# zetanumbers/myraytracer

Measured on AMD Instinct MI355X. Metric: Msamples/s (pixels x spp / s), random-spheres, higher is better.
Workload: dtype f32

## Files before the change

include/myraytracer_amd_debug.h:

```cpp
#ifndef MYRAYTRACER_AMD_DEBUG_H
#define MYRAYTRACER_AMD_DEBUG_H

#include "myraytracer_amd.h"

#ifdef __cplusplus
extern "C" {
#endif

int mrt_debug_srgb8_thresholds(float out[256]);
int mrt_debug_present_encode(mrt_ctx* ctx, const float* rgba, uint32_t width, uint32_t rows, int format, uint32_t flags,
                             uint8_t* out);
int mrt_debug_set_present_copy(mrt_ctx* ctx, int mode);
int mrt_debug_noise_reduce(mrt_ctx* ctx, const float* S, const float* rgba, uint32_t width, uint32_t rows, double K,
                           float threshold, float floor, mrt_noise_report* out, float* tiles_out);
int mrt_debug_denoise(mrt_ctx* ctx, const float* rgba, const float* S, double K, const float* guides, uint32_t width, uint32_t rows,
                      const mrt_denoise_params* params, float* out);
int mrt_debug_denoise_variance(mrt_ctx* ctx, const float* rgba, const float* S, double K, const float* guides, uint32_t width,
                               uint32_t rows, const mrt_denoise_params* params, uint32_t variance, float* out);
int mrt_debug_denoise_mix(mrt_ctx* ctx, const float* rgba, const float* S, double K, const float* guides, uint32_t width,
                          uint32_t rows, const mrt_denoise_params* params, uint32_t variance, const mrt_denoise_mix* mix, float* out);
int mrt_debug_read_guides(mrt_ctx* ctx, float* rays, int32_t* index, float* t, float* normal, float* albedo, size_t cap_pixels);
int mrt_debug_read_gathered_guides(mrt_ctx* root_ctx, float* rays, int32_t* index, float* t, float* normal, float* albedo, size_t cap_pixels);

int mrt_debug_set_gather_per_band(mrt_ctx* root_ctx, int enabled);
// ... 10 lines not shown
                          size_t boxes_cap, uint32_t info[8]);
int mrt_debug_build_boxes_top_down(const mrt_sphere* spheres, size_t n, uint32_t max_levels, uint32_t top_target, int open,
                                   float* boxes_out, size_t boxes_cap, uint32_t info[5]);
int mrt_debug_mfma_scale(double reach, float scale_out[4], uint32_t* neg_k2_bf16_pair_out);
int mrt_debug_build_sweep(const mrt_sphere* spheres, size_t n, const float* force_axis, float axis_out[3], float* records_out,
                          size_t records_cap, uint16_t* mfma_out, size_t mfma_cap, float origin_out[3], double* reach_out);
int mrt_debug_set_sweep_axes(mrt_ctx* ctx, const float* axis);
int mrt_debug_sweep_axes(mrt_ctx* ctx, float axis_out[3]);
int mrt_debug_world_hit(mrt_ctx* ctx, const float* rays, size_t n, int32_t* hit_out, uint32_t* candidates_out,
                        size_t cand_words_per_ray);
int mrt_debug_world_hit_stats(mrt_ctx* ctx, uint64_t out[2]);
int mrt_debug_arith(mrt_ctx* ctx, int mode, const uint32_t bits_range[4], uint64_t count, uint64_t seed, uint64_t out[3]);
int mrt_debug_arith_pairs(mrt_ctx* ctx, const float* x, const float* y, size_t n, uint32_t* out);
int mrt_debug_last_launch(mrt_ctx* ctx, uint32_t out[2]);
int mrt_debug_set_boxes(mrt_ctx* ctx, int mode);
int mrt_debug_sweep_variant(mrt_ctx* ctx);
int mrt_debug_set_frame_batching(mrt_ctx* ctx, int enabled);
int mrt_debug_set_tile_sort(mrt_ctx* ctx, int enabled);
int mrt_debug_sort_tiles(mrt_ctx* ctx, const uint32_t* cost, size_t n_cost, const uint32_t* list, size_t n, uint32_t* order_out);
#define MRT_TILE_ORDER_NONE 0u
#define MRT_TILE_ORDER_INDEX 1u
#define MRT_TILE_ORDER_SORTED 2u
#define MRT_TILE_ORDER_SORTED_LIST 3u
#define MRT_TILE_ORDER_LIST 4u
int mrt_debug_read_tile_schedule(mrt_ctx* ctx, uint32_t* cost_out, uint32_t* order_out, size_t cap, uint32_t* n_out,
                                 uint32_t info_out[4]);
int mrt_debug_set_schedule(mrt_ctx* ctx, uint32_t pilot_spp, int waves_per_cu);
int mrt_debug_lds_layout(uint32_t n_members, uint32_t n_nodes, uint32_t levels, uint32_t n_top_padded, uint32_t out[3]);
int mrt_debug_set_frames_in_flight(mrt_ctx* ctx, int slots);
int mrt_debug_width_policy(int op, const uint32_t workload[6], uint32_t state[7], double util, double rate);
// ... 36 lines not shown
```

myraytracer_amd/_lib.py:

```python
import ctypes as C
import importlib.util
import os
import sys

os.environ.setdefault("GPU_MAX_HW_QUEUES", "20")

_HERE = os.path.dirname(os.path.abspath(__file__))
LIB_PATH = os.environ.get("MRT_LIB_OVERRIDE") or os.path.join(_HERE, "lib", "libmyraytracer_amd.so")

EXPORTS = [
    "mrt_args_default", "mrt_args_resolve_size", "mrt_create", "mrt_destroy", "mrt_set_shard",
    "mrt_set_stream", "mrt_set_world_raw", "mrt_set_world", "mrt_update_spheres", "mrt_pack_world", "mrt_set_camera",
    "mrt_camera_derive", "mrt_set_seeds", "mrt_read_seeds", "mrt_redraw", "mrt_render", "mrt_sync",
    "mrt_reset", "mrt_get_locals", "mrt_set_rng_shuffle", "mrt_set_samples_per_frame", "mrt_set_rng_mode",
    "mrt_frames_done", "mrt_frame_weight", "mrt_frame_shuffle", "mrt_pixel_seed", "mrt_shard_info",
    "mrt_framebuffer_device_ptr", "mrt_read_framebuffer", "mrt_read_counters", "mrt_last_kernel_ms",
    "mrt_kernel_ms_history", "mrt_debug_read_counters", "mrt_debug_wave_log", "mrt_debug_set_tile_sort", "mrt_debug_set_cluster_factor", "mrt_debug_set_hierarchy", "mrt_debug_set_sweep", "mrt_debug_sweep_variant", "mrt_debug_build_hierarchy", "mrt_debug_read_pixel_costs", "mrt_debug_set_schedule", "mrt_debug_mfma_scale", "mrt_debug_build_sweep", "mrt_debug_set_sweep_axes", "mrt_debug_sweep_axes",
    "mrt_last_error", "mrt_status_string", "mrt_abi_version", "mrt_build_id", "mrt_scene_default", "mrt_scene_cover",
    "mrt_scene_stress", "mrt_scene_save", "mrt_scene_load", "mrt_write_pfm", "mrt_write_ppm",
    "mrt_srgb8", "mrt_write_png", "mrt_gather", "mrt_gather_rccl", "mrt_gathered_device_ptr", "mrt_read_gathered",
    "mrt_shard_global_row", "mrt_shard_local_rows", "mrt_unshard_rows", "mrt_debug_last_set_world_ms", "mrt_debug_world_hit", "mrt_debug_world_hit_stats", "mrt_debug_set_frame_batching", "mrt_debug_set_gather_per_band", "mrt_debug_arith", "mrt_debug_arith_pairs", "mrt_debug_set_boxes", "mrt_debug_build_boxes", "mrt_set_draw_counting", "mrt_debug_last_launch", "mrt_debug_set_frames_in_flight", "mrt_debug_lds_layout", "mrt_debug_build_boxes_top_down",
    "mrt_set_wait_timeout", "mrt_get_schedule", "mrt_set_schedule_hint", "mrt_debug_width_policy", "mrt_debug_stream_concurrency", "mrt_debug_wave_log_frame",
    "mrt_present", "mrt_present_acquire", "mrt_present_release", "mrt_set_present_ring", "mrt_debug_srgb8_thresholds",
    "mrt_debug_present_encode", "mrt_debug_set_present_copy",
# ... 5 lines not shown
    "mrt_debug_check_context", "mrt_debug_sort_tiles", "mrt_debug_read_tile_schedule", "mrt_debug_read_hierarchy",
    "mrt_regroup_spheres", "mrt_debug_regroup_info", "mrt_debug_set_regroup_block", "mrt_debug_pool_clusters",
    "mrt_debug_set_camera_masks", "mrt_debug_read_camera_masks", "mrt_debug_read_camera_lists",
    "mrt_temporal_params_default", "mrt_set_temporal", "mrt_get_temporal", "mrt_temporal_step", "mrt_temporal_reset",
    "mrt_read_temporal", "mrt_debug_read_temporal", "mrt_debug_load_temporal",
    "mrt_temporal_response_default", "mrt_set_temporal_response", "mrt_get_temporal_response",
    "mrt_debug_read_temporal_fast", "mrt_debug_load_temporal_fast",
    "mrt_set_gather_noise", "mrt_read_gathered_noise", "mrt_read_gathered_denoised", "mrt_debug_read_gathered_guides",
    "mrt_set_denoise_adaptive", "mrt_get_denoise_adaptive", "mrt_debug_load_accumulation",
    "mrt_auto_regroup_default", "mrt_set_auto_regroup", "mrt_get_auto_regroup", "mrt_read_regroup_stats",
    "mrt_denoise_mix_default", "mrt_set_denoise_mix", "mrt_get_denoise_mix", "mrt_debug_denoise_mix",
    "mrt_update_materials", "mrt_debug_material_shade",
    "mrt_debug_hold", "mrt_debug_hold_stamps",
    "mrt_noise_query_map", "mrt_budget_allocate", "mrt_render_budget",
    "mrt_noise_query_budget", "mrt_read_budget_plan", "mrt_render_planned", "mrt_debug_budget_plan",
]

PRESENT_RGBA8_SRGB, PRESENT_BGRA8_SRGB = 1, 2
PRESENT_FLIP_Y, PRESENT_GATHERED, PRESENT_DENOISED, PRESENT_TEMPORAL, PRESENT_GATHERED_DENOISED = 1, 2, 8, 16, 32
ACQUIRE_NEWEST, ACQUIRE_OLDEST = 0, 1
TILE_ORDER_KINDS = ("none", "index", "sorted", "sorted-list", "list")
DENOISE_VAR_ACCUMULATED, DENOISE_VAR_PREFILTERED, DENOISE_VAR_SPATIAL_EARLY = 0, 1, 2
TILE_MAP_MAX_REL, TILE_MAP_SUM_S = 0, 1
TILE_MAP_KINDS = ("max_rel", "sum_s")
MATERIALS_RESTART_HISTORY = 1
HOLD_CONTEXT, HOLD_SLOT, HOLD_PRESENT, HOLD_NOISE = 0, 1, 2, 3
HOLD_MAX_TICKS = 50_000_000


class MrtArgs(C.Structure):
# ... 260 lines not shown
        "mrt_write_png": (i32, [C.c_char_p, vp, u32, u32]),
        "mrt_gather": (i32, [P(vp), u32, u32]),
        "mrt_gather_rccl": (i32, [vp, vp, u32]),
        "mrt_gathered_device_ptr": (vp, [vp]),
        "mrt_read_gathered": (i32, [vp, vp, sz]),
        "mrt_shard_global_row": (u32, [u32, u32, u32]),
        "mrt_shard_local_rows": (u32, [u32, u32]),
        "mrt_unshard_rows": (i32, [vp, u32, u32, u32, vp]),
        "mrt_debug_last_set_world_ms": (i32, [vp, P(f32)]),
        "mrt_debug_world_hit": (i32, [vp, vp, sz, vp, vp, sz]),
        "mrt_debug_set_frame_batching": (i32, [vp, i32]),
        "mrt_debug_set_gather_per_band": (i32, [vp, i32]),
        "mrt_debug_arith": (i32, [vp, i32, P(u32), u64, u64, P(u64)]),
        "mrt_debug_arith_pairs": (i32, [vp, vp, vp, sz, vp]),
        "mrt_debug_set_boxes": (i32, [vp, i32]),
        "mrt_debug_build_boxes": (i32, [vp, sz, u32, u32, vp, sz, vp]),
        "mrt_set_draw_counting": (i32, [vp, i32]),
        "mrt_debug_last_launch": (i32, [vp, P(u32)]),
        "mrt_debug_world_hit_stats": (i32, [vp, P(u64)]),
        "mrt_debug_set_frames_in_flight": (i32, [vp, i32]),
        "mrt_debug_lds_layout": (i32, [u32, u32, u32, u32, P(u32)]),
        "mrt_debug_build_boxes_top_down": (i32, [vp, sz, u32, u32, i32, vp, sz, vp]),
        "mrt_set_wait_timeout": (i32, [vp, C.c_double]),
        "mrt_get_schedule": (i32, [vp, P(u32)]),
        "mrt_set_schedule_hint": (i32, [vp, u32, u32]),
        "mrt_debug_width_policy": (i32, [i32, P(u32), P(u32), C.c_double, C.c_double]),
        "mrt_debug_stream_concurrency": (i32, [vp, u32, P(f32)]),
        "mrt_debug_wave_log_frame": (i32, [vp, u32, vp, sz, P(sz)]),
        "mrt_present": (i32, [vp, i32, u32]),
        "mrt_present_acquire": (i32, [vp, i32, i32, P(P(C.c_uint8)), P(MrtPresentInfo)]),
# ... 69 lines not shown
```

myraytracer_amd/api.py:

```python
import ctypes as C
import os
from dataclasses import dataclass, field
from typing import List, Optional, Sequence, Tuple

import numpy as np

from . import _lib
from ._lib import MrtArgs, MrtCamera, MrtCameraRaw, MrtCounters, MrtLocals, MrtMaterial, MrtSphere, MrtWorld

LAMBERTIAN, METAL, DIELECTRIC = 1, 2, 3
SPHERE_DTYPE = np.dtype([("center", "<f4", 3), ("radius", "<f4"), ("material_ty", "<i4"),
                         ("albedo", "<f4", 3), ("param", "<f4")])
assert SPHERE_DTYPE.itemsize == C.sizeof(MrtSphere) == 36
MATERIAL_DTYPE = np.dtype([("material_ty", "<i4"), ("albedo", "<f4", 3), ("param", "<f4")])
assert MATERIAL_DTYPE.itemsize == C.sizeof(MrtMaterial) == 20


class MrtError(RuntimeError):
    def __init__(self, status, where, detail=""):
        self.status = status
        name = _lib.load().mrt_status_string(status).decode()
        super().__init__(f"{where}: {name}" + (f" ({detail})" if detail else ""))


# ... 534 lines not shown
        tiles = ((width + 7) // 8) * (rows // 8)
        n, info = C.c_uint32(), (C.c_uint32 * 4)()
        cost, order = np.empty(tiles, np.uint32), np.empty(tiles, np.uint32)
        self._check(self._L.mrt_debug_read_tile_schedule(self._ctx, cost.ctypes.data, order.ctypes.data, tiles, C.byref(n), info),
                    "mrt_debug_read_tile_schedule")
        assert n.value == tiles
        return cost, order[:info[1]].copy(), {"kind": _lib.TILE_ORDER_KINDS[info[0]], "entries": int(info[1]), "pilot": bool(info[2]),
                                              "slot": int(info[3])}

    def debug_set_tile_sort(self, enabled: bool):
        self._check(self._L.mrt_debug_set_tile_sort(self._ctx, int(enabled)), "mrt_debug_set_tile_sort")

    def debug_set_boxes(self, mode):
        self._check(self._L.mrt_debug_set_boxes(self._ctx, 2 if mode is True else int(mode)), "mrt_debug_set_boxes")

    def debug_arith(self, mode: int, bits_range: Sequence[int], count: int = 0, seed: int = 1):
        out = (C.c_uint64 * 3)()
        r = (C.c_uint32 * 4)(*(list(bits_range) + [0, 0, 0, 0])[:4])
        self._check(self._L.mrt_debug_arith(self._ctx, mode, r, count, seed, out), "mrt_debug_arith")
        return int(out[0]), int(out[1]), int(out[2])

    def debug_arith_pairs(self, x: np.ndarray, y: np.ndarray) -> np.ndarray:
        x = np.ascontiguousarray(x, np.float32)
        y = np.ascontiguousarray(y, np.float32)
        assert x.shape == y.shape and x.ndim == 1
        out = np.zeros((len(x), 6), np.uint32)
        self._check(self._L.mrt_debug_arith_pairs(self._ctx, x.ctypes.data, y.ctypes.data, len(x), out.ctypes.data), "mrt_debug_arith_pairs")
        return out

    def debug_set_frame_batching(self, enabled):
# ... 543 lines not shown
```

myraytracer_amd/csrc/kernels.hip:

```cpp

#include <hip/hip_runtime.h>
#include "mrt_internal.h"
#include "mrt_device.h"
#include "sweep.h"
#include "blend.h"

#include <type_traits>

namespace mrt {
namespace {

__device__ __forceinline__ float sphere_quadratic(float cx, float cy, float cz, float neg_r2, V3 o, V3 d, float a, float& b, float& c) {
    const float ocx = o.x - cx, ocy = o.y - cy, ocz = o.z - cz;
    b = __builtin_fmaf(ocz, d.z, __builtin_fmaf(ocy, d.y, ocx * d.x));
    c = __builtin_fmaf(ocz, ocz, __builtin_fmaf(ocy, ocy, __builtin_fmaf(ocx, ocx, neg_r2)));
    return __builtin_fmaf(b, b, -(a * c));
}
__device__ __forceinline__ void literal_test(const SphereRec s, uint32_t idx, V3 o, V3 d, float a,
                                             float& t_sup, int32_t& best) {
    float b, c;
    const float disc = sphere_quadratic(s.cx, s.cy, s.cz, s.neg_r2, o, d, a, b, c);
    if (!(disc < 0.0f)) {
        float d_sqrt = __builtin_sqrtf(disc);
        const float t_min = 0.001f;
// ... 69 lines not shown
    return x;
}
__device__ __forceinline__ uint32_t wave_incl_max(uint32_t x) {
#define MRT_DPP_MAX(ctrl, rmask) { const uint32_t y_ = (uint32_t)__builtin_amdgcn_update_dpp(0, (int)x, ctrl, rmask, 0xF, false); x = x < y_ ? y_ : x; }
    MRT_DPP_MAX(0x111, 0xF);
    MRT_DPP_MAX(0x112, 0xF);
    MRT_DPP_MAX(0x114, 0xF);
    MRT_DPP_MAX(0x118, 0xF);
    MRT_DPP_MAX(0x142, 0xA);
    MRT_DPP_MAX(0x143, 0xC);
#undef MRT_DPP_MAX
    return x;
}
constexpr uint32_t kItemWindow = 256;
static_assert(kSmallGenCap * 2u >= kItemWindow * 4u && kSmallGenCap * 2u >= 3u * 64u * 4u, "the small scenes' table and pick_word's reads below the masks");
__device__ __forceinline__ void lds_order() { asm volatile("" ::: "memory"); }
__device__ __forceinline__ uint32_t rank_in(unsigned long long mask) {
    return __builtin_amdgcn_mbcnt_hi((uint32_t)(mask >> 32), __builtin_amdgcn_mbcnt_lo((uint32_t)mask, 0u));
}

constexpr uint32_t kCtrBlock = MRT_COUNTER_BLOCK;
constexpr uint32_t kRingCap = 128;

typedef const KParams __attribute__((address_space(4)))* KArgPtr;
__device__ __forceinline__ KArgPtr cold_args() {
    KArgPtr p = (KArgPtr)__builtin_amdgcn_kernarg_segment_ptr();
    asm volatile("" : "+s"(p));
    return p;
}

// ... 10 lines not shown
    const bool ok_near = !(t_near < t_min) && t_near < 1.0e4f;
    const bool ok_far = !(t_far < t_min) && t_far < 1.0e4f;
    const float t = ok_near ? t_near : t_far;
    return (hq && (ok_near || ok_far)) ? (((unsigned long long)__float_as_uint(t) << 32) | sidx) : kNoHitKey;
}
__device__ __forceinline__ V3 unit_direction(const V3 ndir) {
    const float dd = dot3(ndir, ndir);
    const float nd_min = __builtin_fminf(__builtin_fminf(__builtin_fabsf(ndir.x), __builtin_fabsf(ndir.y)), __builtin_fabsf(ndir.z));
    if (__builtin_expect(__any(!normalize_unscaled_ok(dd, nd_min)), 0)) return normalize3(ndir);
    const Divisor by_len = divisor_of(sqrt_unscaled(dd));
    return v3(div_unscaled(ndir.x, by_len), div_unscaled(ndir.y, by_len), div_unscaled(ndir.z, by_len));
}

constexpr uint32_t kWavesPerGroup = 4;
template <bool COUNT, bool PILOT, bool CTR, int SC, bool MFMA, bool DBG = false>
__global__ void __launch_bounds__(64 * kWavesPerGroup) __attribute__((amdgpu_waves_per_eu(SC == 0 || SC == 3 ? 5 : 4, 8))) render_kernel(const KParams P) {
    constexpr bool SMALL = SC == 0 || SC == 3, QUAD = SC == 2, LISTS = SC == 3;
    typedef typename Ent<SMALL>::type entry_t;
    constexpr uint32_t kIdBits = Ent<SMALL>::id_bits;
    extern __shared__ __attribute__((aligned(16))) unsigned char lds_raw[];
    const uint32_t lane = threadIdx.x & 63u, wave = threadIdx.x >> 6;
    const uint32_t levels = SMALL ? 1u : P.levels;
    const uint32_t nodes_bytes = SMALL ? P.n_nodes * (uint32_t)sizeof(SphereRec) + lds_index_bytes(P.n_members)
                                       : P.box_lds_count * (uint32_t)sizeof(BoxRec);
    unsigned char* const wlds = lds_raw + nodes_bytes + wave * lds_wave_bytes(SMALL, levels, P.gen_cap, P.mask_chunks);
    float4* const rays = reinterpret_cast<float4*>(wlds + lds_off_rays());
    unsigned long long* const best_slots = reinterpret_cast<unsigned long long*>(wlds + lds_off_rays()) + 3;
    uint32_t* const ring = reinterpret_cast<uint32_t*>(wlds + lds_off_ring());
    entry_t* const queues = reinterpret_cast<entry_t*>(wlds + lds_off_queues());
    uint32_t* const masks = reinterpret_cast<uint32_t*>(wlds + lds_off_masks(SMALL, levels, P.gen_cap)) + lane;
    const uint16_t* const index_lds = reinterpret_cast<const uint16_t*>(lds_raw + P.n_nodes * (uint32_t)sizeof(SphereRec));
    if (SMALL) {
// ... 131 lines not shown
            }
            const float o_rel2 = MFMA ? dot3(o_rel, o_rel) : 0.0f;
            bool weird, usable;
            unsigned long long usable_mask = 0ull;
            if constexpr (SMALL) {
                const unsigned long long admitted = __builtin_amdgcn_ballot_w64(a > 0.99999f) & __builtin_amdgcn_ballot_w64(a < 1.00001f) &
                                                    (MFMA ? __builtin_amdgcn_ballot_w64(o_rel2 <= P.mfma_scale[3]) : ~0ull);
                usable_mask = trace_mask & admitted;
                weird = !__builtin_amdgcn_inverse_ballot_w64(admitted);
                usable = __builtin_amdgcn_inverse_ballot_w64(usable_mask);
            } else {
                weird = !(a > 0.99999f && a < 1.00001f) || (MFMA && !(o_rel2 <= P.mfma_scale[3]));
                usable = trace && !weird;
            }
            unsigned long long key0 = kNoHitKey;
            {
                const KArgPtr C = cold_args();
                const uint32_t n_direct = C->n_direct;
                const Divisor by_a = divisor_of(a);
                for (uint32_t j = 0; j < n_direct; j++) {
                    const float cx = C->direct[j].cx, cy = C->direct[j].cy, cz = C->direct[j].cz, nr2 = C->direct[j].neg_r2;
                    const uint32_t sidx = C->direct_index[j];
                    bool hq;
                    const unsigned long long key = sphere_root_key(cx, cy, cz, nr2, sidx, o, d, a, by_a, usable, hq);
                    key0 = key < key0 ? key : key0;
                    if (DBG && hq) atomicOr(P.dbg_cand + (size_t)texel * P.dbg_words + (sidx >> 5), 1u << (sidx & 31u));
                }
                if (!SMALL) usable_mask = __builtin_amdgcn_ballot_w64(usable);
                if (!PILOT) mtests += (unsigned long long)n_direct * (uint32_t)__popcll(usable_mask);
            }
            rays[2u * lane + 0u] = make_float4(o.x, o.y, o.z, d.x);
            rays[2u * lane + 1u] = make_float4(d.y, d.z, __uint_as_float((uint32_t)key0), __uint_as_float((uint32_t)(key0 >> 32)));
            lds_order();
// ... 127 lines not shown
                    for (int q = 0; q < 4; q++) {
                        const unsigned long long mk = hm[q] & on_mask;
                        if (h[q] && on) dst[pushed + rank_in(mk)] = (entry_t)(e0 + (uint32_t)q);
                        pushed += (uint32_t)__popcll(mk);
                    }
                    return pushed;
                };
                if constexpr (SMALL) {
                    uint32_t qn0 = 0;
                    entry_t* const q0 = queues;
                    uint32_t* const starts = reinterpret_cast<uint32_t*>(queues + kQueueCap);
                    const uint32_t* const masks0 = masks - lane;
                    const uint32_t words = (blk_end - blk) / (2u * kChunk);
                    const bool own = rem != 0u;
                    const unsigned long long own_mask = __builtin_amdgcn_ballot_w64(own);
                    if (own_mask != 0ull) {
                        const uint32_t w0 = top;
                        const uint32_t m0 = masks[w0 * 64u];
                        const uint32_t node = blk + w0 * (2u * kChunk) + (own ? 31u - (uint32_t)__builtin_ctz(m0) : 0u);
                        qn0 += members_round(nodes + 4u * node, o, d, a, own, own_mask, (lane << kIdBits) | (4u * node), q0 + qn0);
                        if (!PILOT) mtests += kClusterK * (uint32_t)__popcll(own_mask);
#ifdef MRT_STAMPS
                        rounds_a_++; items_a_ += (uint32_t)__popcll(own_mask);
#endif
                        lds_order();
                        MRT_WALK_STAMP(2);
                        while (qn0 >= 64u) root_round(q0, qn0);
                    }
                    const uint32_t rest = rem - (own ? 1u : 0u);
                    const uint32_t incl = wave_incl_scan(rest);
                    const uint32_t total_rem = (uint32_t)__builtin_amdgcn_readlane((int)incl, 63);
                    const uint32_t start_entry = rest != 0u ? ((incl - rest) << 6) | lane : 0xFFFFFFFFu;
                    uint32_t carry = 0u;
                    auto pick_word = [&](auto NW, const uint32_t owner, const uint32_t r, uint32_t& sel, uint32_t& r_in) -> uint32_t {
                        constexpr int n = decltype(NW)::value;
                        const uint32_t* const mo = masks0 + (int32_t)(words - (uint32_t)n) * 64 + owner;
                        uint32_t cnt = 0u, above = 0u, below = 0u;
                        bool found = false;
                        sel = 0u;
#pragma unroll
                        for (int i = n - 1; i >= 0; i--) {
                            const uint32_t m = mo[i * 64];
                            sel = found ? sel : m;
                            above = found ? above : cnt;
                            cnt += (uint32_t)__builtin_popcount(m);
                            found = r < cnt;
                            below += found ? 0u : 1u;
                        }
                        r_in = r - above;
                        return blk + (words - 1u - below) * (2u * kChunk);
                    };
                    for (uint32_t base = 0; base < total_rem; base += kItemWindow) {
#pragma unroll
                        for (uint32_t i = 0; i < kItemWindow; i += 64u) starts[i + lane] = 0u;
                        lds_order();
                        if ((start_entry >> 6) - base < kItemWindow) starts[(start_entry >> 6) - base] = start_entry;
                        lds_order();
                        const uint32_t window_end = total_rem - base < kItemWindow ? total_rem : base + kItemWindow;
                        for (uint32_t g0 = base; g0 < window_end; g0 += 64u) {
                            const uint32_t take = total_rem - g0 < 64u ? total_rem - g0 : 64u;
                            const bool act = lane < take;
                            const unsigned long long act_mask = take < 64u ? (1ull << take) - 1ull : ~0ull;
                            uint32_t e = starts[g0 - base + lane];
                            e = wave_incl_max(e < carry ? carry : e);
                            carry = (uint32_t)__builtin_amdgcn_readlane((int)e, 63);
                            const uint32_t owner = e & 63u;
                            const uint32_t r = g0 + (act ? lane : take - 1u) - (e >> 6) + 1u;
                            uint32_t sel, r_in;
                            const uint32_t first = words <= 4u ? pick_word(IC<4>{}, owner, r, sel, r_in) : pick_word(IC<8>{}, owner, r, sel, r_in);
                            for (uint32_t trip = 0; trip < 31u && __any(r_in != 0u); trip++) {
                                if (r_in != 0u) { sel &= sel - 1u; r_in--; }
                            }
                            const uint32_t node = first + 31u - (uint32_t)__builtin_ctz(sel);
                            V3 ro, rd;
                            fetch_ray(owner, ro, rd);
                            MRT_WALK_STAMP(6);
                            qn0 += members_round(nodes + 4u * node, ro, rd, dot3(rd, rd), act, act_mask, (owner << kIdBits) | (4u * node), q0 + qn0);
                            if (!PILOT) mtests += kClusterK * take;
#ifdef MRT_STAMPS
                            rounds_a_++; items_a_ += take;
#endif
                            lds_order();
// ... 547 lines not shown
    if (cap < n_waves) n_waves = cap;
    const uint32_t want = n_waves < p.n_tiles ? n_waves : p.n_tiles;
    return dim3((want + kWavesPerGroup - 1) / kWavesPerGroup);
}
template <bool COUNT, bool PILOT, bool CTR, bool DBG>
static void launch_render_kernel(const KParams& p, uint32_t n_waves, hipStream_t st) {
    uint32_t lds;
    const dim3 grid = persistent_grid(p, n_waves, &lds), block(64 * kWavesPerGroup);
    auto with_sweep = [&](auto sc) {
        auto go = [&](auto mfma) {
            hipLaunchKernelGGL((render_kernel<COUNT, PILOT, CTR, decltype(sc)::value, decltype(mfma)::value != 0, DBG>), grid, block, lds, st, p);
        };
        if (p.use_mfma != 0) go(IC<1>{}); else go(IC<0>{});
    };
    if (scene_is_small(p.n_members)) {
        if constexpr (!DBG) { if (p.cam_lists != nullptr) { with_sweep(IC<3>{}); return; } }
        with_sweep(IC<0>{});
    }
    else if (p.box_quad != 0) with_sweep(IC<2>{});
    else with_sweep(IC<1>{});
}

int launch_render(const KParams& p, bool pilot, uint32_t n_waves, void* stream, uint32_t* which) {
    if (which) *which = 0xFFFFFFFFu;
    if (p.n_tiles == 0 || n_waves == 0) return 0;
    hipStream_t st = (hipStream_t)stream;
    const bool small = scene_is_small(p.n_members);
    const bool ctr = p.locals.rng_mode == MRT_RNG_COUNTER;
    const bool mfma = p.use_mfma != 0, quad = p.box_quad != 0;
    if (which) *which = ((!pilot && p.count_draws) ? 1u : 0u) | (pilot ? 2u : 0u) | (ctr ? 4u : 0u) | (small ? 8u : 0u) | (mfma ? 16u : 0u) |
                        ((!small && quad) ? 32u : 0u) | (p.cam_lists != nullptr ? 64u : 0u);
    if (pilot) {
// ... 49 lines not shown
```

myraytracer_amd/csrc/mrt_ctx.h:

```cpp
#pragma once
#include <hip/hip_runtime_api.h>

#include <chrono>
#include <string>
#include <vector>

#include "mrt_internal.h"
#include "width_policy.h"

struct mrt_ctx {
    int device = 0;
    mrt_args args{};
    uint64_t seed = 0;
    mrt_locals locals{};
    uint32_t frames_done = 0;

    uint32_t shard_rank = 0, shard_world = 1;
    uint32_t local_bands = 0;

    mrt_world world{};
    bool have_world = false;
    uint32_t n_spheres = 0, n_padded = 0;
    mrt_camera_raw cam_raw{};

// ... 18 lines not shown
    size_t regroup_words = 0;
    uint32_t auto_updates = 0;
    uint32_t* d_cam_masks = nullptr;
    size_t cam_mask_entries = 0;
    uint32_t* cam_lists() const { return d_cam_masks ? d_cam_masks + 4 * cam_mask_entries : nullptr; }
    uint64_t cam_mask_gen = 1, cam_mask_built = 0, cam_mask_seen = 0;
    bool cam_masks_on = true, cam_masks_in_force = false;
    uint32_t cam_prefer = 0;
    bool cam_lists_in_force = false;
    mrt::BoxRec* d_boxes = nullptr;
    mrt::BoxRec* d_boxes_open = nullptr;
    uint32_t box_cluster_first = 0, box_cluster_parent_first = 0;
    bool box_quad = false;
    float box_kc = 0.0f;
    int boxes_mode = 1;
    float cluster_factor = 8.0f;
    uint32_t max_levels = mrt::kMaxLevels, top_target = 0;
    uint32_t levels = 1, n_nodes = 0, n_members = 0;
    uint32_t level_base[mrt::kMaxLevels] = {0, 0, 0, 0};
    uint32_t n_direct = 0, direct_first = 0;
    mrt::SphereRec direct[mrt::kMaxDirect] = {};
    uint32_t direct_index[mrt::kMaxDirect] = {};
    float* d_vec4 = nullptr;
    float* d_f32 = nullptr;
    int32_t* d_i32 = nullptr;
    uint32_t* d_seeds = nullptr;
    float* d_fb[2] = {nullptr, nullptr};
    int target = 0;
    unsigned long long* d_counters = nullptr;
    bool count_draws = true;
// ... 226 lines not shown
```

myraytracer_amd/csrc/mrt_internal.h:

```cpp
#pragma once
#include <stdint.h>
#include "../../include/myraytracer_amd.h"
#include "../../include/myraytracer_amd_debug.h"

namespace mrt {

constexpr uint32_t kBandRows = 8;
constexpr uint32_t kTileW = 8;
constexpr uint32_t kChunk = 16;
constexpr uint32_t kGroup = 8;
constexpr uint32_t kClusterK = 4;
constexpr uint32_t kMaxSpheres = 1u << 20;
constexpr uint32_t kMaxLevels = 4;
constexpr float kBoundStretch = 1.0001f;
constexpr double kBoundInflate = 1.015;
constexpr uint32_t kMaxFrameBatch = 32;
constexpr uint32_t kQueueCap = 320;
constexpr uint32_t kSmallGenCap = 576;
constexpr uint32_t kStackReserve = 16;
constexpr uint32_t kMaxDirect = 4;
constexpr uint32_t kCamMaskRecords = 128;
constexpr uint32_t kCamListCap = 8;
constexpr uint32_t kCamListOverflow = 0xFFFFFFFFu;
inline bool scene_is_small(uint32_t n_members) { return n_members <= 1024u; }
// ... 44 lines not shown
    const uint32_t* tile_order;
    uint32_t* tile_queue;
    uint32_t tiles_x, n_tiles;
    uint32_t pilot_spp;
    uint32_t* tile_cost;
    void* pix_acc;
    uint32_t n_blocks, pix_stride, queue_layers, lane_frames;
    uint32_t layer_shuffle[kMaxFrameBatch][4];
    unsigned long long* wave_log;
    const float* dbg_rays;
    int32_t* dbg_hit;
    uint32_t* dbg_cand;
    uint32_t dbg_words;
    const uint32_t* cam_masks;
    const uint32_t* cam_lists;
};

void set_global_error(const char* msg);

int launch_render(const KParams& p, bool pilot, uint32_t n_waves, void* stream, uint32_t* which = nullptr);
int launch_finalize(const KParams& p, void* stream, float* noise_s = nullptr);
int launch_debug_world_hit(const KParams& p, uint32_t n_waves, void* stream);
int render_waves_per_cu(int* out);
void render_lds_layout(const KParams& p, uint32_t out[2]);
uint32_t render_resident_waves(const KParams& p);
uint32_t large_scene_stack_cap(uint32_t mask_chunks, uint32_t box_lds_count);
uint32_t large_scene_box_lds_count(uint32_t n_top_padded, uint32_t levels, uint32_t mask_chunks, uint32_t cap);
constexpr uint32_t kBoxLdsCap = 1024;
int launch_sort_tiles(const uint32_t* cost, uint32_t* order, uint32_t* scratch, uint32_t n_tiles, void* stream);
int launch_sort_tile_list(const uint32_t* cost, const uint32_t* list, uint32_t* order, uint32_t* scratch, uint32_t n, void* stream);
// ... 272 lines not shown
```

myraytracer_amd/csrc/world.cpp:

```cpp
#include <algorithm>
#include <cmath>
#include <cstring>

#include "mrt_ctx.h"
#include "hierarchy.h"

using mrt::fail, mrt::free_world, mrt::Hierarchy, mrt::build_hierarchy, mrt::build_sweep_operand, mrt::boxes_top_down, mrt::pack_boxes, mrt::kMfmaSlack, mrt::fill_scene_params;

namespace {

bool finite_in_range(float v, float lim) { return std::isfinite(v) && std::fabs(v) <= lim; }

bool use_matrix_core_sweep(const mrt_ctx* c) {
    if (c->sweep_mode == 2) return true;
    if (c->sweep_mode == 1 || !c->mfma_scene_ok) return false;
    double o2 = 0.0;
    for (int k = 0; k < 3; k++) {
        const double d = (double)c->mfma_axis[k] * ((c->cam_raw.mode ? (double)c->cam_raw.origin[k] : 0.0) - (double)c->mfma_origin[k]);
        o2 += d * d;
    }
    return kMfmaSlack * o2 <= 0.1 * c->mfma_r2_ref;
}

mrt::RefitArgs refit_args(const mrt_ctx* c) {
// ... 114 lines not shown
                const double u = (double)c->mfma_axis[k] * c->cam_raw.ru[k], v = (double)c->mfma_axis[k] * c->cam_raw.rv[k];
                u2 += u * u; v2 += v * v;
            }
            lens = std::sqrt(u2) + std::sqrt(v2);
        }
        mfma_scales(std::max(c->mfma_reach, std::sqrt(cam_d2) + lens), p.mfma_scale, &p.mfma_neg_k2_pair);
    }
    p.levels = c->levels; p.n_nodes = c->n_nodes; p.n_members = c->n_members;
    p.box_lds_count = mrt::scene_is_small(c->n_members) ? 0u : mrt::large_scene_box_lds_count(c->n_padded, c->levels, p.mask_chunks, mrt::kBoxLdsCap);
    p.gen_cap = mrt::scene_is_small(c->n_members) ? mrt::kSmallGenCap : mrt::large_scene_stack_cap(p.mask_chunks, p.box_lds_count);
    for (uint32_t k = 0; k < mrt::kMaxLevels; k++) p.level_base[k] = c->level_base[k];
    p.boxes = c->boxes_mode == 0 ? c->d_boxes_open : c->d_boxes;
    p.box_cluster_first = c->box_cluster_first; p.box_cluster_parent_first = c->box_cluster_parent_first;
    p.box_quad = c->box_quad ? 1u : 0u;
    p.box_kc = c->box_kc;
    p.n_direct = c->n_direct; p.direct_first = c->direct_first;
    for (uint32_t k = 0; k < mrt::kMaxDirect; k++) { p.direct[k] = c->direct[k]; p.direct_index[k] = c->direct_index[k]; }
    p.cus = c->cus;
    p.spheres = c->d_spheres; p.clusters = c->d_clusters; p.nodes = c->d_nodes; p.top_mfma = c->d_top_mfma; p.member_index = c->d_member_index; p.vec4_data = c->d_vec4; p.shade = c->d_shade; p.f32_data = c->d_f32; p.i32_data = c->d_i32;
}

}

extern "C" {

int mrt_set_world_raw(mrt_ctx* c, const void* world, size_t world_bytes, const float* vec4, size_t n_vec4,
                      const float* f32, size_t n_f32, const int32_t* i32, size_t n_i32) {
    if (!c || !world) return MRT_ERR_INVALID_ARG;
    const auto t_begin = std::chrono::steady_clock::now();
    if (world_bytes != MRT_WORLD_BYTES_REFERENCE && world_bytes != sizeof(mrt_world))
// ... 485 lines not shown
                std::memset(cand_out + i * cand_words, 0, cand_words * sizeof(uint32_t));
                std::memcpy(cand_out + i * cand_words, cand.data() + i * words, need_words * sizeof(uint32_t));
            }
    }
    cleanup();
    if (e != hipSuccess) return fail(c, MRT_ERR_HIP, "mrt_debug_world_hit: read-back failed: %s", hipGetErrorString(e));
    return MRT_OK;
}

int mrt_debug_set_boxes(mrt_ctx* c, int mode) {
    if (!c || mode < 0 || mode > 2) return MRT_ERR_INVALID_ARG;
    c->boxes_mode = mode;
    return MRT_OK;
}

int mrt_debug_sweep_variant(mrt_ctx* c) {
    if (!c || !c->have_world) return 0;
    return use_matrix_core_sweep(c) ? 2 : 1;
}

int mrt_debug_set_hierarchy(mrt_ctx* c, uint32_t max_levels, uint32_t top_target) {
    if (!c || max_levels < 1 || max_levels > mrt::kMaxLevels) return MRT_ERR_INVALID_ARG;
    c->max_levels = max_levels;
    c->top_target = top_target;
    return MRT_OK;
}

int mrt_debug_lds_layout(uint32_t n_members, uint32_t n_nodes, uint32_t levels, uint32_t n_top_padded, uint32_t out[3]) {
    if (!out || levels < 1 || levels > mrt::kMaxLevels) return MRT_ERR_INVALID_ARG;
    mrt::KParams p;
// ... 13 lines not shown
```

Measured before the change: 18830.

## Choose per-wave walk plan between in-lane and cooperative member rounds

For small scenes without camera lists (SC==0), each wave now decides whether to run the in-lane first member round. It skips that round when running it would not cut the number of cooperative 64-item rounds, using one inclusive scan of the remaining counts for the decision. A debug knob forces plans with 0, 1 or 2 in-lane rounds through new kernel variants, and a Python cost model script evaluates those plans. The change adds kernel instantiations, a scan before the own-round and some register pressure, and it alters the rank arithmetic for the cooperative distribution.

```diff
diff --git a/experiments/walk_plan_model.py b/experiments/walk_plan_model.py
--- /dev/null
+++ b/experiments/walk_plan_model.py
@@ -0,0 +1,109 @@
+#!/usr/bin/env python3
+import os
+import re
+import sys
+
+import numpy as np
+
+ROOT = os.path.dirname(os.path.dirname(os.path.abspath(__file__)))
+sys.path.insert(0, ROOT)
+sys.path.insert(0, os.path.join(ROOT, "tests"))
+sys.path.insert(0, os.path.join(ROOT, "experiments"))
+import myraytracer_amd as M
+from oracle import pyoracle as O
+from common import to_oracle_spheres
+from cand_hist import candidates, sweep_records
+
+_SRC = open(os.path.join(ROOT, "myraytracer_amd", "csrc", "kernels.hip")).read()
+C_LANE, C_LANE1, C_COOP = (int(re.search(rf"\b{n} = (\d+)u", _SRC).group(1)) for n in ("kWalkLaneCost", "kWalkLane1Cost", "kWalkCoopCost"))
+MEASURED = {"c3": (108.0, 1.20), "c2": (2.02 * 40.6, 1.02)}
+
+
+def ray_counts(glass):
+    rng = np.random.default_rng(5)
+    n_rays = 4096
+    sc, cam = M.scene_cover(1, glass)
+    packed = O.pack_world(to_oracle_spheres(O, sc))
+    lf, la = np.array(cam.lookfrom, float), np.array(cam.lookat, float)
+    fw = (la - lf) / np.linalg.norm(la - lf)
+    right = np.cross(fw, np.array(cam.vup, float))
+    right /= np.linalg.norm(right)
+    up = np.cross(right, fw)
+    th = np.tan(np.radians(cam.vfov_deg) / 2)
+    u = rng.uniform(-1, 1, n_rays) * th * 16 / 9
+    v = rng.uniform(-1, 1, n_rays) * th
+    d = fw[None] + u[:, None] * right[None] + v[:, None] * up[None]
+    d /= np.linalg.norm(d, axis=1, keepdims=True)
+    rays = np.concatenate([np.repeat(lf[None], n_rays, 0), d], 1).astype(np.float32)
+    centers = np.asarray(sc["center"], float).reshape(-1, 3)
+    radii = np.asarray(sc["radius"], float)
+    rec, org, D = sweep_records(sc)
+    per_depth = []
+    for depth in range(12):
+        if len(rays) == 0:
+            break
+        per_depth.append(candidates(rays, rec, org, D))
+        hit, t, _, _ = O.world_hit_batch(packed, rays)
+        ok = hit >= 0
+        r = rays[ok].astype(float)
+        p = r[:, :3] + t[ok, None] * r[:, 3:]
+        n = (p - centers[hit[ok]]) / radii[hit[ok], None]
+        s = rng.normal(size=n.shape)
+        s /= np.linalg.norm(s, axis=1, keepdims=True)
+        nd = n + s
+        nd /= np.linalg.norm(nd, axis=1, keepdims=True)
+        rays = np.concatenate([p, nd], 1).astype(np.float32)
+    return per_depth[0], np.concatenate(per_depth[1:]), len(rec)
+
+
+def plan_costs(t, k1, k2):
+    coop = [(t + 63) // 64, (t - k1 + 63) // 64, (t - k1 - k2 + 63) // 64]
+    lane = [np.zeros_like(t), np.where(k1 > 0, C_LANE, 0), np.where(k1 > 0, C_LANE, 0) + np.where(k2 > 0, C_LANE1, 0)]
+    return np.stack([l + c * C_COOP for l, c in zip(lane, coop)]), np.stack(coop)
+
+
+def report(name, counts, n_records):
+    items, rounds = MEASURED[name]
+    rng = np.random.default_rng(11)
+    p = min(1.0, items / (64.0 * counts.mean()))
+    n_waves = 20000
+    lanes = rng.choice(counts, (n_waves, 64)) * (rng.random((n_waves, 64)) < p)
+    t, k1, k2 = lanes.sum(1), (lanes >= 1).sum(1), (lanes >= 2).sum(1)
+    busy = t > 0
+    t, k1, k2 = t[busy], k1[busy], k2[busy]
+    cost, coop = plan_costs(t, k1, k2)
+    print(f"== {name}: {n_records} top records ({n_records // 32} mask words), {counts.mean():.2f} candidates per walking ray, busy lanes per wave {64 * p:.1f} (fitted: p = {p:.3f})")
+    print(f"   T {t.mean():.1f} (measured {items:.1f}), K {k1.mean():.1f}, K2 {k2.mean():.1f}; cooperative rounds per iteration under today's plan "
+          f"{coop[1].mean():.2f} (measured {rounds:.2f}), with no in-lane round {coop[0].mean():.2f}, with two {coop[2].mean():.2f}")
+    print("   T - K over a multiple of 64 by:   " + "  ".join(f"{lo}-{lo + 15}: {100 * np.mean(((t - k1 - 1) % 64 >= lo) & ((t - k1 - 1) % 64 < lo + 16) & (t > k1)):.0f} %" for lo in (0, 16, 32, 48)))
+    print("   distribution of (T, K, K2), percentiles 10 / 50 / 90:  " + "  ".join(f"{n} {np.percentile(v, 10):.0f} / {np.percentile(v, 50):.0f} / {np.percentile(v, 90):.0f}" for n, v in (("T", t), ("K", k1), ("K2", k2))))
+    fixed = cost[1]
+    best01, arg01 = cost[:2].min(0), cost[:2].argmin(0)
+    arg012 = arg01.copy()
+    c2_better = (cost[2] < best01) | ((cost[2] == best01) & (coop[2] < np.where(arg01 == 1, coop[1], coop[0])))
+    arg012[c2_better] = 2
+    best012 = np.where(c2_better, cost[2], best01)
+    print("   | plan | walk VALU per busy iteration | saving | blocks with 0 / 1 / 2 in-lane rounds |")
+    print("   |---|---|---|---|")
+    for label, c, a in (("today's fixed plan (one in-lane round)", fixed, np.ones_like(arg01)), ("best of {0, 1}", best01, arg01), ("best of {0, 1, 2}", best012, arg012)):
+        share = " / ".join(f"{100 * np.mean(a == k):.0f} %" for k in (0, 1, 2))
+        print(f"   | {label} | {c.mean():.0f} | {fixed.mean() - c.mean():.0f} | {share} |")
+    s01, s012 = fixed.mean() - best01.mean(), fixed.mean() - best012.mean()
+    print(f"   the second in-lane round's share of the total saving: {100 * (s012 - s01) / max(s012, 1e-9):.0f} %")
+    return abs(t.mean() / items - 1), abs(coop[1].mean() / rounds - 1), (s012 - s01) / max(s012, 1e-9)
+
+
+def main():
+    print(f"costs (kernels.hip): in-lane round 0 {C_LANE}, in-lane round 1 {C_LANE1}, cooperative round {C_COOP} VALU instructions")
+    cam3, bounce3, n3 = ray_counts(True)
+    e_items, e_rounds, share = report("c3", bounce3, n3)
+    cam2, bounce2, n2 = ray_counts(False)
+    report("c2", np.concatenate([cam2, bounce2]), n2)
+    ok = e_items < 0.03 and e_rounds < 0.05
+    print(f"check (C3): items within {100 * e_items:.1f} %, cooperative rounds within {100 * e_rounds:.1f} % of the committed profile: {'ok' if ok else 'NOT reproduced'}")
+    print(f"decision: the second in-lane round gives {100 * share:.0f} % of C3's modelled saving; the bar for building it is 25 %")
+    return 0 if ok else 1
+
+
+if __name__ == "__main__":
+    sys.exit(main())
diff --git a/include/myraytracer_amd_debug.h b/include/myraytracer_amd_debug.h
--- a/include/myraytracer_amd_debug.h
+++ b/include/myraytracer_amd_debug.h
@@ -48,6 +48,7 @@
 int mrt_debug_arith_pairs(mrt_ctx* ctx, const float* x, const float* y, size_t n, uint32_t* out);
 int mrt_debug_last_launch(mrt_ctx* ctx, uint32_t out[2]);
 int mrt_debug_set_boxes(mrt_ctx* ctx, int mode);
+int mrt_debug_set_walk_plan(mrt_ctx* ctx, int mode);
 int mrt_debug_sweep_variant(mrt_ctx* ctx);
 int mrt_debug_set_frame_batching(mrt_ctx* ctx, int enabled);
 int mrt_debug_set_tile_sort(mrt_ctx* ctx, int enabled);
diff --git a/myraytracer_amd/_lib.py b/myraytracer_amd/_lib.py
--- a/myraytracer_amd/_lib.py
+++ b/myraytracer_amd/_lib.py
@@ -43,6 +43,7 @@
     "mrt_debug_hold", "mrt_debug_hold_stamps",
     "mrt_noise_query_map", "mrt_budget_allocate", "mrt_render_budget",
     "mrt_noise_query_budget", "mrt_read_budget_plan", "mrt_render_planned", "mrt_debug_budget_plan",
+    "mrt_debug_set_walk_plan",
 ]
 
 PRESENT_RGBA8_SRGB, PRESENT_BGRA8_SRGB = 1, 2
@@ -333,6 +334,7 @@
         "mrt_debug_arith": (i32, [vp, i32, P(u32), u64, u64, P(u64)]),
         "mrt_debug_arith_pairs": (i32, [vp, vp, vp, sz, vp]),
         "mrt_debug_set_boxes": (i32, [vp, i32]),
+        "mrt_debug_set_walk_plan": (i32, [vp, i32]),
         "mrt_debug_build_boxes": (i32, [vp, sz, u32, u32, vp, sz, vp]),
         "mrt_set_draw_counting": (i32, [vp, i32]),
         "mrt_debug_last_launch": (i32, [vp, P(u32)]),
diff --git a/myraytracer_amd/api.py b/myraytracer_amd/api.py
--- a/myraytracer_amd/api.py
+++ b/myraytracer_amd/api.py
@@ -572,6 +572,9 @@
     def debug_set_boxes(self, mode):
         self._check(self._L.mrt_debug_set_boxes(self._ctx, 2 if mode is True else int(mode)), "mrt_debug_set_boxes")
 
+    def debug_set_walk_plan(self, mode: int):
+        self._check(self._L.mrt_debug_set_walk_plan(self._ctx, int(mode)), "mrt_debug_set_walk_plan")
+
     def debug_arith(self, mode: int, bits_range: Sequence[int], count: int = 0, seed: int = 1):
         out = (C.c_uint64 * 3)()
         r = (C.c_uint32 * 4)(*(list(bits_range) + [0, 0, 0, 0])[:4])
diff --git a/myraytracer_amd/csrc/kernels.hip b/myraytracer_amd/csrc/kernels.hip
--- a/myraytracer_amd/csrc/kernels.hip
+++ b/myraytracer_amd/csrc/kernels.hip
@@ -107,6 +107,10 @@
 }
 constexpr uint32_t kItemWindow = 256;
 static_assert(kSmallGenCap * 2u >= kItemWindow * 4u && kSmallGenCap * 2u >= 3u * 64u * 4u, "the small scenes' table and pick_word's reads below the masks");
+constexpr uint32_t kWalkLaneCost = 143u, kWalkLane1Cost = 175u, kWalkCoopCost = 248u;
+static_assert(0u < kWalkLaneCost && kWalkLaneCost <= kWalkLane1Cost && kWalkLane1Cost < kWalkCoopCost,
+              "the plan's choice is written as a comparison of cooperative rounds");
+constexpr bool kWalkPlanAuto = true;
 __device__ __forceinline__ void lds_order() { asm volatile("" ::: "memory"); }
 __device__ __forceinline__ uint32_t rank_in(unsigned long long mask) {
     return __builtin_amdgcn_mbcnt_hi((uint32_t)(mask >> 32), __builtin_amdgcn_mbcnt_lo((uint32_t)mask, 0u));
@@ -147,8 +151,10 @@
 
 constexpr uint32_t kWavesPerGroup = 4;
 template <bool COUNT, bool PILOT, bool CTR, int SC, bool MFMA, bool DBG = false>
-__global__ void __launch_bounds__(64 * kWavesPerGroup) __attribute__((amdgpu_waves_per_eu(SC == 0 || SC == 3 ? 5 : 4, 8))) render_kernel(const KParams P) {
-    constexpr bool SMALL = SC == 0 || SC == 3, QUAD = SC == 2, LISTS = SC == 3;
+__global__ void __launch_bounds__(64 * kWavesPerGroup) __attribute__((amdgpu_waves_per_eu(SC == 0 || SC >= 3 ? 5 : 4, 8))) render_kernel(const KParams P) {
+    constexpr bool PLAN = SC >= 4;
+    constexpr bool SMALL = SC == 0 || SC == 3 || PLAN, QUAD = SC == 2, LISTS = SC == 3 || SC == 5;
+    constexpr bool PLANNED = PLAN || (kWalkPlanAuto && SC == 0);
     typedef typename Ent<SMALL>::type entry_t;
     constexpr uint32_t kIdBits = Ent<SMALL>::id_bits;
     extern __shared__ __attribute__((aligned(16))) unsigned char lds_raw[];
@@ -310,9 +316,11 @@
                 usable = trace && !weird;
             }
             unsigned long long key0 = kNoHitKey;
+            uint32_t walk_forced = 0u;
             {
                 const KArgPtr C = cold_args();
                 const uint32_t n_direct = C->n_direct;
+                if constexpr (PLAN) walk_forced = C->walk_plan;
                 const Divisor by_a = divisor_of(a);
                 for (uint32_t j = 0; j < n_direct; j++) {
                     const float cx = C->direct[j].cx, cy = C->direct[j].cy, cz = C->direct[j].cz, nr2 = C->direct[j].neg_r2;
@@ -470,7 +478,19 @@
                     const uint32_t words = (blk_end - blk) / (2u * kChunk);
                     const bool own = rem != 0u;
                     const unsigned long long own_mask = __builtin_amdgcn_ballot_w64(own);
-                    if (own_mask != 0ull) {
+                    uint32_t plan_k = 1u, incl_rem = 0u, total_items = 0u;
+                    unsigned long long two_mask = 0ull;
+                    if constexpr (PLANNED) {
+                        incl_rem = wave_incl_scan(rem);
+                        total_items = (uint32_t)__builtin_amdgcn_readlane((int)incl_rem, 63);
+                        if constexpr (PLAN) {
+                            two_mask = __builtin_amdgcn_ballot_w64(rem >= 2u);
+                            plan_k = walk_forced - 1u;
+                        } else {
+                            plan_k = ((total_items - (uint32_t)__popcll(own_mask) + 63u) >> 6) < ((total_items + 63u) >> 6) ? 1u : 0u;
+                        }
+                    }
+                    if (plan_k >= 1u && own_mask != 0ull) {
                         const uint32_t w0 = top;
                         const uint32_t m0 = masks[w0 * 64u];
                         const uint32_t node = blk + w0 * (2u * kChunk) + (own ? 31u - (uint32_t)__builtin_ctz(m0) : 0u);
@@ -483,9 +503,23 @@
                         MRT_WALK_STAMP(2);
                         while (qn0 >= 64u) root_round(q0, qn0);
                     }
-                    const uint32_t rest = rem - (own ? 1u : 0u);
-                    const uint32_t incl = wave_incl_scan(rest);
-                    const uint32_t total_rem = (uint32_t)__builtin_amdgcn_readlane((int)incl, 63);
+                    uint32_t rest, incl, total_rem;
+                    if constexpr (PLANNED) {
+                        const unsigned long long m1 = plan_k >= 1u ? own_mask : 0ull, m2 = plan_k >= 2u ? two_mask : 0ull;
+                        uint32_t below = rank_in(m1);
+                        uint32_t taken = __builtin_amdgcn_inverse_ballot_w64(m1) ? 1u : 0u;
+                        if constexpr (PLAN) {
+                            below = __builtin_amdgcn_mbcnt_hi((uint32_t)(m2 >> 32), __builtin_amdgcn_mbcnt_lo((uint32_t)m2, below));
+                            taken = rem < plan_k ? rem : plan_k;
+                        }
+                        rest = rem - taken;
+                        incl = incl_rem - taken - below;
+                        total_rem = total_items - (uint32_t)__popcll(m1) - (uint32_t)__popcll(m2);
+                    } else {
+                        rest = rem - (own ? 1u : 0u);
+                        incl = wave_incl_scan(rest);
+                        total_rem = (uint32_t)__builtin_amdgcn_readlane((int)incl, 63);
+                    }
                     const uint32_t start_entry = rest != 0u ? ((incl - rest) << 6) | lane : 0xFFFFFFFFu;
                     uint32_t carry = 0u;
                     auto pick_word = [&](auto NW, const uint32_t owner, const uint32_t r, uint32_t& sel, uint32_t& r_in) -> uint32_t {
@@ -506,6 +540,23 @@
                         r_in = r - above;
                         return blk + (words - 1u - below) * (2u * kChunk);
                     };
+                    if constexpr (PLAN) {
+                    if (plan_k >= 2u && two_mask != 0ull) {
+                        const bool two = __builtin_amdgcn_inverse_ballot_w64(two_mask);
+                        uint32_t sel, r_in;
+                        const uint32_t first = words <= 4u ? pick_word(IC<4>{}, lane, 1u, sel, r_in) : pick_word(IC<8>{}, lane, 1u, sel, r_in);
+                        sel = r_in != 0u ? sel & (sel - 1u) : sel;
+                        const uint32_t node = two ? first + 31u - (uint32_t)__builtin_ctz(sel) : blk;
+                        qn0 += members_round(nodes + 4u * node, o, d, a, two, two_mask, (lane << kIdBits) | (4u * node), q0 + qn0);
+                        if (!PILOT) mtests += kClusterK * (uint32_t)__popcll(two_mask);
+#ifdef MRT_STAMPS
+                        rounds_a_++; items_a_ += (uint32_t)__popcll(two_mask);
+#endif
+                        lds_order();
+                        MRT_WALK_STAMP(2);
+                        while (qn0 >= 64u) root_round(q0, qn0);
+                    }
+                    }
                     for (uint32_t base = 0; base < total_rem; base += kItemWindow) {
 #pragma unroll
                         for (uint32_t i = 0; i < kItemWindow; i += 64u) starts[i + lane] = 0u;
@@ -521,7 +572,7 @@
                             e = wave_incl_max(e < carry ? carry : e);
                             carry = (uint32_t)__builtin_amdgcn_readlane((int)e, 63);
                             const uint32_t owner = e & 63u;
-                            const uint32_t r = g0 + (act ? lane : take - 1u) - (e >> 6) + 1u;
+                            const uint32_t r = g0 + (act ? lane : take - 1u) - (e >> 6) + plan_k;
                             uint32_t sel, r_in;
                             const uint32_t first = words <= 4u ? pick_word(IC<4>{}, owner, r, sel, r_in) : pick_word(IC<8>{}, owner, r, sel, r_in);
                             for (uint32_t trip = 0; trip < 31u && __any(r_in != 0u); trip++) {
@@ -1099,8 +1150,8 @@
         if (p.use_mfma != 0) go(IC<1>{}); else go(IC<0>{});
     };
     if (scene_is_small(p.n_members)) {
-        if constexpr (!DBG) { if (p.cam_lists != nullptr) { with_sweep(IC<3>{}); return; } }
-        with_sweep(IC<0>{});
+        if constexpr (!DBG) { if (p.cam_lists != nullptr) { if (p.walk_plan != 0u) with_sweep(IC<5>{}); else with_sweep(IC<3>{}); return; } }
+        if (p.walk_plan != 0u) with_sweep(IC<4>{}); else with_sweep(IC<0>{});
     }
     else if (p.box_quad != 0) with_sweep(IC<2>{});
     else with_sweep(IC<1>{});
diff --git a/myraytracer_amd/csrc/mrt_ctx.h b/myraytracer_amd/csrc/mrt_ctx.h
--- a/myraytracer_amd/csrc/mrt_ctx.h
+++ b/myraytracer_amd/csrc/mrt_ctx.h
@@ -56,6 +56,7 @@
     bool box_quad = false;
     float box_kc = 0.0f;
     int boxes_mode = 1;
+    int walk_plan = 0;
     float cluster_factor = 8.0f;
     uint32_t max_levels = mrt::kMaxLevels, top_target = 0;
     uint32_t levels = 1, n_nodes = 0, n_members = 0;
diff --git a/myraytracer_amd/csrc/mrt_internal.h b/myraytracer_amd/csrc/mrt_internal.h
--- a/myraytracer_amd/csrc/mrt_internal.h
+++ b/myraytracer_amd/csrc/mrt_internal.h
@@ -82,6 +82,7 @@
     uint32_t dbg_words;
     const uint32_t* cam_masks;
     const uint32_t* cam_lists;
+    uint32_t walk_plan;
 };
 
 void set_global_error(const char* msg);
diff --git a/myraytracer_amd/csrc/world.cpp b/myraytracer_amd/csrc/world.cpp
--- a/myraytracer_amd/csrc/world.cpp
+++ b/myraytracer_amd/csrc/world.cpp
@@ -152,6 +152,7 @@
     p.box_cluster_first = c->box_cluster_first; p.box_cluster_parent_first = c->box_cluster_parent_first;
     p.box_quad = c->box_quad ? 1u : 0u;
     p.box_kc = c->box_kc;
+    p.walk_plan = (uint32_t)c->walk_plan;
     p.n_direct = c->n_direct; p.direct_first = c->direct_first;
     for (uint32_t k = 0; k < mrt::kMaxDirect; k++) { p.direct[k] = c->direct[k]; p.direct_index[k] = c->direct_index[k]; }
     p.cus = c->cus;
@@ -667,6 +668,12 @@
     return MRT_OK;
 }
 
+int mrt_debug_set_walk_plan(mrt_ctx* c, int mode) {
+    if (!c || mode < 0 || mode > 3) return MRT_ERR_INVALID_ARG;
+    c->walk_plan = mode;
+    return MRT_OK;
+}
+
 int mrt_debug_sweep_variant(mrt_ctx* c) {
     if (!c || !c->have_world) return 0;
     return use_matrix_core_sweep(c) ? 2 : 1;
```

Result: no change. 18810 (-0.1%).
